# magicat777/Audio-Analyzer-OMEGA

Hardware: AMD Instinct MI355X
Metric: audio frames/sec (multi-res FFT + LUFS + TruePeak) at 1/2/4/8 MI355X (higher is better)
Workload: dtype f32; 1 GPU; cfg2: 256 stereo frames x 16384 samples per GPU; MRFFT 16k/8k/4k/1k + combine(512) + K-weighted LUFS + 4x true peak + meter aggregates; channel_frames_per_gpu=512, frame_samples=16384, target_bins=512, parallelism=frames sharded over 1 GPU(s)

## Files before the change

audio-analyzer-omega_amd/csrc/capi_batch.cpp:

```cpp

#include "batch_plan.hpp"
#include "host.hpp"

namespace {

constexpr int kChunkFrames = kMeterChunk;

int get_kw_tab(omega_ctx* c, int M, int L, BiquadTab** out) {
  const auto key = std::make_pair(M, L);
  auto it = c->kw_tabs.find(key);
  if (it != c->kw_tabs.end()) {
    *out = it->second;
    return 0;
  }
  const double fs = c->cfg.sample_rate;
  std::vector<BiquadTab> t = {make_biquad_tab(butter2(38.0, fs, true), L),
                              make_biquad_tab(butter2(1500.0, fs, true), L)};
  BiquadTab* d = nullptr;
  int r = upload(c, &d, t);
  if (r) return r;
  c->kw_tabs[key] = d;
  *out = d;
  return 0;
}
int get_kw_tab(omega_ctx* c, int M, BiquadTab** out) { return get_kw_tab(c, M, kw_chunk(M), out); }

hipError_t tp_launch(int W, const SpectralParams& sp, hipStream_t s) {
  if (W == 16384 || W == 8192) return launch_truepeak_rf(W, sp, s);
  return launch_truepeak(W, sp, s);
}

SpectralParams spectral_params(omega_ctx* c) {
  SpectralParams p{};
  p.tp_phases = 0xE;
  p.C = c->cfg.n_channels;
  p.n_res = c->cfg.n_res;
  p.rf_sizes = c->rf_sizes;
  for (int r = 0; r < p.n_res; ++r) {
    ResParam& q = p.res[r];
    q.n = c->cfg.res[r].fft_size;
    q.offset = c->cfg.frame_size - q.n;
    q.win = c->d_win[r];
    q.wgt = c->d_wgt[r];
    q.ent_begin = c->ent_begin[r];
    q.ent_end = c->ent_end[r];
    q.cw = (float)c->cfg.res[r].weight;
    q.low_band = c->ent_jmax[r] < 256;
    q.pair_lo = c->pair_lo[r];
    q.pair_hi = c->pair_hi[r];
  }
  p.ent = c->d_ent;
  p.T = c->cfg.target_bins;
  p.rot = c->d_rot;
  for (int l = 0; l < kMaxLog2; ++l) p.tw[l] = c->d_tw[l];
  return p;
}

bool aligned8(const void* p) { return ((uintptr_t)p & 7) == 0; }

std::vector<MeterPrepParams> meter_chunks(omega_ctx* c, const float* lufs, const float* tp, int64_t n_frames,
                                          double* out) {
  const int C = c->cfg.n_channels;
  std::vector<MeterPrepParams> v;
  for (int64_t f0 = 0; f0 < n_frames; f0 += kChunkFrames) {
    const int64_t nf = std::min<int64_t>(kChunkFrames, n_frames - f0);
    const int a = c->cur, b = c->cur ^ 1;
    MeterPrepParams p{};
    p.lufs = lufs + f0 * C;
    p.tp = tp + f0 * C;
    p.n_frames = nf;
    p.C = C;
    p.hist_l_in = c->d_hist_l[a];
    p.hist_t_in = c->d_hist_t[a];
    p.n_l_in = c->d_nl[a];
    p.n_t_in = c->d_nt[a];
    p.skeys_in = c->d_skeys[a];
    p.n_s_in = c->d_ns[a];
    p.t0_in = c->d_t0[a];
    p.hist_l_out = c->d_hist_l[b];
    p.hist_t_out = c->d_hist_t[b];
    p.n_l_out = c->d_nl[b];
    p.n_t_out = c->d_nt[b];
    p.skeys_out = c->d_skeys[b];
    p.n_s_out = c->d_ns[b];
    p.t0_out = c->d_t0[b];
    p.HL = c->HL;
    p.HT = c->HT;
    p.mom_len = c->cfg.momentary_len;
    p.short_len = c->cfg.short_len;
    p.int_len = c->cfg.integrated_len;
    p.peak_len = c->cfg.peak_len;
    p.poll_limit = c->poll_limit;
    p.err_word = c->d_err;
    p.gate = (float)c->cfg.gate_lufs;
    p.core = c->d_core[a];
    p.ext = c->d_ext[a];
    p.n_core = c->d_ncore[a];
    p.n_ext = c->d_next[a];
    p.gcount = c->d_gcount[a];
    p.gsum = c->d_gsum[a];
// ... 836 lines not shown
```

audio-analyzer-omega_amd/csrc/host.hpp:

```cpp
#pragma once

#include <hip/hip_runtime.h>

#include <algorithm>
#include <cmath>
#include <complex>
#include <cstdarg>
#include <cstdio>
#include <cstdlib>
#include <cstring>
#include <exception>
#include <map>
#include <new>
#include <string>
#include <vector>

#include "../../include/omega.h"
#include "design.hpp"
#include "params.hpp"

namespace omega {
hipError_t launch_mrfft(const SpectralParams& p, hipStream_t s);
hipError_t launch_mrfft_independent(const SpectralParams& p, hipStream_t s);
hipError_t launch_truepeak(int W, const SpectralParams& p, hipStream_t s);
// ... 188 lines not shown
  bool use_graph = false;
  int layout = 3;
  unsigned* d_kw_done = nullptr;
  unsigned kw_issued = 0;
  unsigned q_issued = 0;
  unsigned tp_issued = 0;
  unsigned prep_issued = 0;
  unsigned seg_issued = 0;
  unsigned lt_issued = 0;
  unsigned* tp_count_to = nullptr;
  bool side_meters = false;
  unsigned seg_par[2] = {0, 0};
  bool pipe = false;
  bool pend = false;
  MeterPrepParams pend_mq{};
  int pend_nq = 0, pend_par = 0;
  int stage_par = 0;
  unsigned* d_tail = nullptr;
  unsigned tail_issued = 0;
  unsigned long long* d_mirror = nullptr;
  unsigned mirror_gen = 0;
  int tail_ok = 0;
  hipStream_t bs[2] = {nullptr, nullptr};
  hipEvent_t ev_in = nullptr, ev_done[2] = {nullptr, nullptr};
  unsigned bs_idx = 0;
  int last_bs = 0;
  bool unjoined = false;
  bool bs_shared = false;
  std::vector<std::pair<const char*, size_t>> prev_span;
  unsigned* h_err = nullptr;
  unsigned* d_err = nullptr;
  int poll_limit = 1 << 22;
  float* d_lufs_scr = nullptr;
  int64_t lufs_scr_cap = 0;
  bool res_independent = false;
  hipEvent_t ev_kw = nullptr;
  struct GraphEntry {
    std::vector<uint64_t> key;
    hipGraph_t graph;
    hipGraphExec_t exec;
  };
  std::vector<GraphEntry> graphs;
  char err[512] = {};
  float2* d_tw[kMaxLog2] = {};

  float2* d_rot = nullptr;
  float* d_win[kMaxRes] = {};
  float* d_wgt[kMaxRes] = {};
  CombEnt* d_ent = nullptr;
  int ent_begin[kMaxRes] = {}, ent_end[kMaxRes] = {};
  int pair_lo[kMaxRes] = {}, pair_hi[kMaxRes] = {};
  int ent_jmax[kMaxRes] = {};
  std::map<std::pair<int, int>, BiquadTab*> kw_tabs;
  int rf_sizes = 1 << 14;
  std::map<std::pair<int, int>, float*> windows;
  std::map<int, float2*> rots;
  std::map<std::pair<int, int>, float4*> wgens;
  int* d_own_off = nullptr;
  int* d_own_rj = nullptr;
  float* d_own_frac = nullptr;
  std::map<int, std::pair<double*, std::pair<int, int>>> chroma_mats;
  double chroma_df = 0.0;
  struct ChromaTab {
    int n_bins = 0, lo = 0, hi = 0;
    double df = 0.0;
    float4* w4 = nullptr;
    float* w1 = nullptr;
    unsigned short* perm = nullptr;
    int* goff = nullptr;
    float* rec = nullptr;
  } ctab;
  int n_cu = 0;
  DrumState drum;
  PostState post;
  VuState vu;
  TransientState tr;
  PitchState pitch;
  HarmonicState harm;
  GenreState genre;
  HipHopState hiphop;
  PhaseState phase;
  RoomState room;
  VoiceState voice;
  TdetectState tdetect;
  BassZoomState basszoom;
  W64Stage* w64[4] = {};
  struct AnyPlan {
    std::vector<int> radix;
    float2* tw = nullptr;
    double2* tw64 = nullptr;
    float2* rot = nullptr;
  };
  std::map<int, AnyPlan> any_plans;
  float2* d_any = nullptr;
  int64_t any_cap = 0;
  double* d_w64 = nullptr;
  int64_t w64_cap = 0;
  float* d_hist_l[2] = {};
  float* d_hist_t[2] = {};
  int* d_nl[2] = {};
  int* d_nt[2] = {};
  int cur = 0;
  unsigned long long* d_skeys[2] = {};
  int* d_ns[2] = {};
  uint32_t* d_t0[2] = {};
  float* d_core[2] = {nullptr, nullptr};
  MeterExt* d_ext[2] = {nullptr, nullptr};
// ... 275 lines not shown
```

audio-analyzer-omega_amd/csrc/params.hpp:

```cpp
#pragma once
#include <hip/hip_runtime.h>
#include <stdint.h>

namespace omega {

constexpr int kMaxRes = 4;
constexpr int kMaxLog2 = 15;

__device__ __forceinline__ float tp_db(float peak) {
  return peak < 1e-10f ? -100.0f : (float)(20.0 * log10((double)peak));
}

struct alignas(16) CombEnt {
  int tm, j;
  float c0, c1;
};

struct ResParam {
  int n;
  int offset;
  const float* win;
  const float* wgt;
  float* mag_out;
  int ent_begin, ent_end;
  float cw;
  int low_band;
  int pair_lo, pair_hi;
};

struct SpectralParams {
  const float* x;
  int64_t frame_stride, chan_stride;
  int C;
  int64_t n_cf;
  int n_res;
  ResParam res[kMaxRes];
  const CombEnt* ent;
  int T;
  float* comb_out;
  float* tp_out;
  const float2* rot;
  int tp_phases;
  const float2* tw[kMaxLog2];
  int rf_sizes;
  unsigned* tp_done;
  float* tp_copy;
};

struct BiquadTab {
  float b0, a1, a2, B0, B1;
  float zi0, zi1;
  float h0[64], h1[64];
  float pw[64][4];
  float g0[64], g1[64];
};

constexpr int kPwl = 96;
constexpr int kw_threads(int M) { return M / 32 < 64 ? 64 : (M / 32 > 512 ? 512 : M / 32); }
constexpr int kw_chunk(int M) { return M / kw_threads(M); }

struct KWeightParams {
  const float* x;
  int64_t frame_stride, chan_stride;
  int C;
  int64_t n_cf;
  const BiquadTab* hp;
  const BiquadTab* shelf;
  float* lufs_out;
  float* weighted_out;
// ... 537 lines not shown
```

audio-analyzer-omega_amd/csrc/regfft.hpp:

```cpp
#pragma once
#include "fft.hpp"

namespace omega {

__device__ constexpr float kCos128[16] = {
    1.000000000e+00f, 9.987954562e-01f, 9.951847267e-01f, 9.891765100e-01f, 9.807852804e-01f,
    9.700312532e-01f, 9.569403357e-01f, 9.415440652e-01f, 9.238795325e-01f, 9.039892931e-01f,
    8.819212643e-01f, 8.577286100e-01f, 8.314696123e-01f, 8.032075315e-01f, 7.730104534e-01f,
    7.409511254e-01f};
__device__ constexpr float kSin128[16] = {
    0.000000000e+00f, 4.906767433e-02f, 9.801714033e-02f, 1.467304745e-01f, 1.950903220e-01f,
    2.429801799e-01f, 2.902846773e-01f, 3.368898534e-01f, 3.826834324e-01f, 4.275550934e-01f,
    4.713967368e-01f, 5.141027442e-01f, 5.555702330e-01f, 5.956993045e-01f, 6.343932842e-01f,
    6.715589548e-01f};

__device__ __forceinline__ void wave_lds_sync() {
  asm volatile("s_waitcnt lgkmcnt(0)" ::: "memory");
  __builtin_amdgcn_wave_barrier();
}

__device__ __forceinline__ float lane_xor1(float v) {
  return __int_as_float(__builtin_amdgcn_mov_dpp(__float_as_int(v), 0xB1, 0xF, 0xF, true));
}

// ... 123 lines not shown
    }
  }
  static __device__ __forceinline__ void twiddle_t2(float2 (&v)[16], const float2* t2u) {
    static_for<1, 16>([&](auto k2) { v[k2] = cmul(v[k2], t2u[(k2 - 1) * L]); });
  }

  template <bool SYNC = false, bool LT2 = false>
  static __device__ __forceinline__ void run(float2 (&v)[16], float2* buf, int t, float2 w1, float2 w2,
                                             const float2* t2 = nullptr) {
    run2<SYNC, LT2>(v, buf, t, t, w1, w2, t2);
  }
  template <bool SYNC = false, bool LT2 = false>
  static __device__ __forceinline__ void run2(float2 (&v)[16], float2* buf, int t1, int t, float2 w1, float2 w2,
                                              const float2* t2 = nullptr) {
    dft16(v);
    twiddle(v, w1);
    if constexpr (SYNC) __syncthreads();
    {
      float2* b = buf + t1;
      static_for<0, 16>([&](auto k1) { b[P1 * k1] = v[k1]; });
    }
    __syncthreads();
    {
      const int u = t % L, k1 = t / L;
      const float2* b = buf + P1 * k1 + u;
      static_for<0, 16>([&](auto r) { v[r] = b[L * r]; });
      dft16(v);
      if constexpr (LT2)
        twiddle_t2(v, t2 + u);
      else
        twiddle(v, w2);
      float2* bw = buf + P2R * k1 + u;
      static_for<0, 16>([&](auto k2) { bw[P2C * k2] = v[k2]; });
    }
    wave_lds_sync();
    if constexpr (L == 16) {
      const int k2 = t & 15, k1 = t >> 4;
      const float2* b = buf + P2R * k1 + P2C * k2;
      static_for<0, 16>([&](auto r) { v[r] = b[r]; });
      dft16(v);
    } else {
      const int q = t & 1, k2 = (t >> 1) & 15, k1 = t >> 5;
      const float2* b = buf + P2R * k1 + P2C * k2 + q;
      static_for<0, 16>([&](auto r) { v[r] = b[2 * r]; });
      dft16(v);
      static_for<0, 16>([&](auto m) {
        const float2 tw = twc<m + 16, 32>(v[m]);
        v[m] = make_float2(q ? tw.x : v[m].x, q ? tw.y : v[m].y);
      });
      lane_pair_fmac(v, q ? 1.f : -1.f);
    }
  }

  template <bool SYNC = false, bool LT2 = false>
  static __device__ __forceinline__ void run_low(float2 (&v)[16], float2* buf, int t, float2 w1, float2 w2,
                                                 const float2* t2 = nullptr) {
    static_assert(L == 32, "the two-band pass 3 is the K = 8192 plan");
    dft16(v);
    twiddle(v, w1);
    if constexpr (SYNC) __syncthreads();
    {
      float2* b = buf + t;
      static_for<0, 16>([&](auto k1) { b[P1 * k1] = v[k1]; });
    }
    __syncthreads();
    {
      const int u = t % L, k1 = t / L;
      const float2* b = buf + P1 * k1 + u;
      static_for<0, 16>([&](auto r) { v[r] = b[L * r]; });
      dft16(v);
      if constexpr (LT2)
        twiddle_t2(v, t2 + u);
      else
        twiddle(v, w2);
      float2* bw = buf + P2R * k1 + u;
      static_for<0, 16>([&](auto k2) { bw[P2C * k2] = v[k2]; });
    }
    wave_lds_sync();
    const int q = t & 1, k2 = (t >> 1) & 15, k1 = t >> 5;
    {
      const float2* b = buf + P2R * k1 + P2C * k2 + q;
      static_for<0, 16>([&](auto r) { v[r] = b[2 * r]; });
    }
    float2 f0 = v[0], f15 = v[0];
    static_for<1, 16>([&](auto r) {
      f0 = cadd(f0, v[r]);
      f15 = cadd(f15, twc<15 * r, 16>(v[r]));
    });
    const float2 g = twc<15, 32>(f15);
    const float2 send = q ? f0 : f15;
    const float2 recv = make_float2(lane_xor1(send.x), lane_xor1(send.y));
    const float2 out = q ? csub(recv, g) : cadd(f0, recv);
    __syncthreads();
    buf[s3o(t) + (q ? o3o(15) : 0)] = out;
    __syncthreads();
  }

  template <bool LT2 = false>
  static __device__ __forceinline__ void run_half(float2 (&v)[16], float* bf, int t, float2 w1, float2 w2,
                                                  const float2* t2 = nullptr) {
    static_assert(L == 16, "the half-buffer plan is K = 4096");
    dft16(v);
    twiddle(v, w1);
    const int u = t % L, k1 = t / L;
    {
      float* b = bf + t;
      static_for<0, 16>([&](auto j) { b[P1 * j] = v[j].x; });
    }
    __syncthreads();
    {
      const float* b = bf + P1 * k1 + u;
      static_for<0, 16>([&](auto r) { v[r].x = b[L * r]; });
    }
    __syncthreads();
    {
      float* b = bf + t;
      static_for<0, 16>([&](auto j) { b[P1 * j] = v[j].y; });
    }
    __syncthreads();
    {
      const float* b = bf + P1 * k1 + u;
      static_for<0, 16>([&](auto r) { v[r].y = b[L * r]; });
    }
    dft16(v);
    if constexpr (LT2)
      twiddle_t2(v, t2 + u);
    else
      twiddle(v, w2);
    {
      float* bw = bf + P2R * k1 + u;
      static_for<0, 16>([&](auto j) { bw[P2C * j] = v[j].x; });
    }
    wave_lds_sync();
    const int k2 = t & 15, k1b = t >> 4;
    const float* br = bf + P2R * k1b + P2C * k2;
    static_for<0, 16>([&](auto r) { v[r].x = br[r]; });
    {
      float* bw = bf + P2R * k1 + u;
      static_for<0, 16>([&](auto j) { bw[P2C * j] = v[j].y; });
    }
    wave_lds_sync();
    static_for<0, 16>([&](auto r) { v[r].y = br[r]; });
    dft16(v);
  }
  template <bool IM>
  static __device__ __forceinline__ void store_spectrum_half(const float2 (&v)[16], float* bf, int t) {
    float* b = bf + s3o(t);
    static_for<0, 16>([&](auto m) { b[o3o(m)] = IM ? v[m].y : v[m].x; });
// ... 10 lines not shown
```

audio-analyzer-omega_amd/csrc/rfkern.hip:

```cpp
#include <cstdlib>

#include "stamps.hpp"

namespace omega {
OMEGA_STAMPS_DECL
OMEGA_WGTRACE_DECL
OMEGA_MARKS_DECL
}

#include "kw.hpp"
#include "meter_query.hpp"
#include "regfft.hpp"
#include "spectral.hpp"

namespace omega {

template <int K>
constexpr size_t t2_offset() { return (RegFFT<K>::kSlots + 8) * sizeof(float2) + 64; }
template <int K>
constexpr size_t lds_bytes() { return t2_offset<K>() + RegFFT<K>::kT2 * sizeof(float2); }
template <int K>
__device__ __forceinline__ float2* t2_table(char* smem) { return reinterpret_cast<float2*>(smem + t2_offset<K>()); }

template <int NTH>
// ... 81 lines not shown
      const float2 a = bo[FFT::o3(r)];
      float2 b = bm[FFT::o3(15 - r)];
      if constexpr (K == 8192 && r == 8) {
        if (t == 0) b = a;
      }
      float2 xk, xkk;
      untangle(a, b, twc<r, 32>(wm), xk, xkk);
      if constexpr (r == 0) {
        if (t == 0) {
          xn = a.x - a.y;
          xk = make_float2(a.x + a.y, 0.f);
        }
      }
      v[r] = xk;
    });
  }
  float2 y[16];
  static_for<0, 16>([&](auto r) { y[r] = v[r]; });
  const float2 hz = make_float2(wm.y, wm.x);
  float fmx = 0.f;
  const int lane = tid & 63;
  const int mir_addr = 4 * ((t == 0 || t == NTH / 2) ? lane : lane ^ 63);
  OMEGA_STAMP(4);
#pragma unroll 1
  for (int P = 1; P <= 3; ++P) {
    int tl = t, tidl = tid;
    float2 w1l = w1, w2l = w2, rhol = rho, hzl = hz;
    asm volatile("" : "+v"(tl), "+v"(tidl), "+v"(w1l.x), "+v"(w1l.y), "+v"(w2l.x), "+v"(w2l.y));
    asm volatile("" : "+v"(rhol.x), "+v"(rhol.y), "+v"(hzl.x), "+v"(hzl.y));
    static_for<0, 16>([&](auto r) {
      const float2 rk = cmul(rhol, make_float2(kCos128[r], kSin128[r]));
      y[r] = cmul(y[r], rk);
    });
    if (!((p.tp_phases >> P) & 1)) continue;
    OMEGA_STAMP(1 + 4 * P);
    const float cp = P == 1 ? 7.071067812e-01f : (P == 2 ? 0.f : -7.071067812e-01f);
    OMEGA_STAMP(2 + 4 * P);
    static_for<0, 16>([&](auto r) {
      const float2 m = y[15 - r];
      float2 yp = make_float2(__int_as_float(__builtin_amdgcn_ds_bpermute(mir_addr, __float_as_int(m.x))),
                              -__int_as_float(__builtin_amdgcn_ds_bpermute(mir_addr, __float_as_int(m.y))));
      if constexpr (r == 0) {
        if (tl == 0) yp = make_float2(xn * cp, 0.f);
      } else {
        if (tl == 0) yp = cconj(y[16 - r]);
      }
      const float2 g = twc<-r, 32>(hzl);
      const float2 S = cadd(y[r], yp), D = csub(y[r], yp);
      v[r] = make_float2(fmaf(g.x, D.x, fmaf(-g.y, D.y, S.x)), fmaf(-g.x, D.y, fmaf(-g.y, D.x, -S.y)));
    });
    OMEGA_STAMP(3 + 4 * P);
    FFT::template run2<true, true>(v, buf, tl, tidl, w1l, w2l, t2);
    max3_abs16(fmx, v);
#if defined(OMEGA_EXP_STALL)
    asm volatile("s_sleep %0" ::"i"(OMEGA_EXP_STALL));
#endif
#if defined(OMEGA_EXP_VALU)
    {
      float d0 = fmx, d1 = mx, d2 = fmx + 1.f, d3 = mx + 1.f;
      asm volatile(".rept %4\n v_fma_f32 %0, %0, %5, %6\n v_fma_f32 %1, %1, %5, %6\n"
                   " v_fma_f32 %2, %2, %5, %6\n v_fma_f32 %3, %3, %5, %6\n .endr"
                   : "+v"(d0), "+v"(d1), "+v"(d2), "+v"(d3)
                   : "i"(OMEGA_EXP_VALU), "v"(0.5f), "v"(0.25f));
    }
#endif
    OMEGA_STAMP(4 + 4 * P);
  }
  const float peak = block_max<NTH>(fmaxf(mx, fmx * (0.5f / K)), red, tid);
  if (tid == 0) {
    const float db = tp_db(peak);
    if (p.tp_done) {
      __hip_atomic_store(reinterpret_cast<unsigned*>(p.tp_out + cf), __float_as_uint(db), __ATOMIC_RELAXED,
                         __HIP_MEMORY_SCOPE_AGENT);
      asm volatile("s_waitcnt vmcnt(0)" ::: "memory");
      __hip_atomic_fetch_add(p.tp_done, 1u, __ATOMIC_RELAXED, __HIP_MEMORY_SCOPE_AGENT);
    } else {
      p.tp_out[cf] = db;
    }
    if (p.tp_copy) p.tp_copy[cf] = db;
  }
}

template <int K>
__global__ __launch_bounds__(K / 16, 4) void truepeak_rf_kernel(SpectralParams p) {
  extern __shared__ __attribute__((aligned(16))) char smem[];
  OMEGA_WG_BEGIN();
  truepeak_rf_body<K>(p, blockIdx.x, threadIdx.x, smem);
  OMEGA_WG_END(1);
}

template <int K>
__device__ __forceinline__ void mrfft_rf_body(const SpectralParams& p, int r, int64_t cf, int t, char* smem) {
  using FFT = RegFFT<K>;
  constexpr int NTH = FFT::NTH, M = 2 * K;
  float2* buf = reinterpret_cast<float2*>(smem);
  const int64_t f = cf / p.C, c = cf % p.C;
  const ResParam& rp = p.res[r];
  const float2* x2 = reinterpret_cast<const float2*>(p.x + f * p.frame_stride + c * p.chan_stride + rp.offset);
  const float2* __restrict__ twK = p.tw[ilog2(K)];
  const float2* __restrict__ twM = p.tw[ilog2(M)];
  float2 v[16];
  const float2 w1 = twK[t], w2b = twK[16 * (t % FFT::L)];
  const float2 wm = twM[t];
  float2* t2 = t2_table<K>(smem);
  FFT::fill_t2(t2, twK, t);
  asm volatile("" ::: "memory");
  const float2* w2 = reinterpret_cast<const float2*>(rp.win);
  static_for<0, 16>([&](auto q) {
    const float2 a = x2[t + NTH * q], w = w2[t + NTH * q];
    v[q] = make_float2(a.x * w.x, a.y * w.y);
  });
  const int e0 = rp.ent_begin + t;
  CombEnt ent{};
  if (p.comb_out && e0 < rp.ent_end) ent = p.ent[e0];
  bool low = false;
  if constexpr (K == 8192) low = !rp.mag_out && rp.low_band;
  if (low) {
    if constexpr (K == 8192) FFT::template run_low<false, true>(v, buf, t, w1, w2b, t2);
  } else {
    FFT::template run<false, true>(v, buf, t, w1, w2b, t2);
    __syncthreads();
    FFT::store_spectrum(v, buf, t);
    __syncthreads();
  }
  if (!rp.mag_out) {
    if (!p.comb_out) return;
    auto mag_at = [&](int j) -> float {
      const float2 a = buf[FFT::a3(j == K ? 0 : j)];
      if (j == 0) return fabsf(a.x + a.y);
      if (j == K) return fabsf(a.x - a.y);
      if (j == K / 2) return cabs(a);
      const float2 b = buf[FFT::a3(K - j)];
      float2 xk, xkk;
      untangle(a, b, twM[j], xk, xkk);
      return cabs(xk);
    };
    float* o = p.comb_out + cf * p.T;
    auto apply = [&](const CombEnt& en) {
      const int tt = en.tm & 0xFFFFFF, op = en.tm >> 24;
      if (op == 2) {
        o[tt] = 0.f;
        return;
      }
      const float val = fmaf(en.c1, mag_at(en.j + 1), en.c0 * mag_at(en.j));
      if (op == 0)
        o[tt] = val;
      else
        o[tt] += val;
    };
    if (e0 < rp.ent_end) apply(ent);
    for (int e = e0 + NTH; e < rp.ent_end; e += NTH) apply(p.ent[e]);
    return;
  }
  float mg[16];
  float mnyq = 0.f;
  {
    const float2* bo = buf + FFT::s3(t);
    const float2* bm = buf + FFT::s3m(t);
    static_for<0, 16>([&](auto q) {
      const float2 a = bo[FFT::o3(q)];
      float2 b = bm[FFT::o3(15 - q)];
      if constexpr (K == 8192 && q == 8) {
        if (t == 0) b = a;
      }
      float2 xk, xkk;
      untangle(a, b, twc<q, 32>(wm), xk, xkk);
      mg[q] = cabs(xk);
      if constexpr (q == 0) {
        if (t == 0) {
          mg[0] = fabsf(a.x + a.y);
          mnyq = fabsf(a.x - a.y);
        }
      }
    });
  }
  if (rp.mag_out) {
    float* o = rp.mag_out + cf * (K + 1);
    const float* __restrict__ wgt = rp.wgt;
    static_for<0, 16>([&](auto q) { o[t + NTH * q] = mg[q] * wgt[t + NTH * q]; });
    if (t == 0) o[K] = mnyq * wgt[K];
  }
  if (!p.comb_out) return;
  float* mag = reinterpret_cast<float*>(smem);
  __syncthreads();
  static_for<0, 16>([&](auto q) { mag[t + NTH * q] = mg[q]; });
  if (t == 0) mag[K] = mnyq;
  __syncthreads();
  float* o = p.comb_out + cf * p.T;
  auto apply = [&](const CombEnt& en) {
    const int tt = en.tm & 0xFFFFFF, op = en.tm >> 24;
    const float val = fmaf(en.c1, mag[en.j + 1], en.c0 * mag[en.j]);
    if (op == 0)
      o[tt] = val;
    else if (op == 1)
      o[tt] += val;
    else
      o[tt] = 0.f;
  };
  if (e0 < rp.ent_end) apply(ent);
  for (int e = e0 + NTH; e < rp.ent_end; e += NTH) apply(p.ent[e]);
}

template <int K>
__global__ __launch_bounds__(K / 16, 4) void mrfft_rf_kernel(SpectralParams p, int r) {
  extern __shared__ __attribute__((aligned(16))) char smem[];
  OMEGA_WG_BEGIN();
  mrfft_rf_body<K>(p, r, blockIdx.x, threadIdx.x, smem);
  OMEGA_WG_END(2);
}

OMEGA_STAMPS_GETTER(omega_debug_rf_stamps)
OMEGA_WGTRACE_GETTER(omega_debug_wgtrace)
OMEGA_MARKS_GETTER(omega_debug_marks_batch)

hipError_t launch_mrfft_rf(int n, const SpectralParams& p, int r, hipStream_t s) {
  const dim3 grid((unsigned)p.n_cf);
  if (n == 16384) {
    hipLaunchKernelGGL(mrfft_rf_kernel<8192>, grid, dim3(512), lds_bytes<8192>(), s, p, r);
  } else if (n == 8192) {
    hipLaunchKernelGGL(mrfft_rf_kernel<4096>, grid, dim3(256), lds_bytes<4096>(), s, p, r);
  } else {
    return hipErrorInvalidValue;
  }
  return hipGetLastError();
}

constexpr int kSpecRfThreads = 256;
#ifndef OMEGA_SPEC_WGS
#define OMEGA_SPEC_WGS 5
#endif
constexpr int kSpecRfWgs = OMEGA_SPEC_WGS;
constexpr int kSpecRfPeakWords = 12;
template <int K>
struct SpecRfLds {
  static constexpr size_t kT2Off = RegFFT<K>::kSlots * sizeof(float);
  static constexpr size_t kXform = kT2Off + RegFFT<K>::kT2 * sizeof(float2);
  static constexpr size_t kPartOff = ((K + 1) * sizeof(float) + 15) / 16 * 16;
  static constexpr size_t kClsOff = kPartOff + 240 * 5 * sizeof(float);
  static constexpr size_t kRedOff = kClsOff + 12 * 5 * sizeof(double);
  static constexpr size_t kFlagOff = (kRedOff + (RegFFT<K>::NTH / 64) * sizeof(float) + 15) / 16 * 16;
  static constexpr int kFlagWords = 2 * 64 * kSpecRfPeakWords / 4;
  static constexpr size_t kPost = kFlagOff + kFlagWords * sizeof(unsigned);
  static constexpr size_t kBytes = kXform > kPost ? kXform : kPost;
  static_assert((kBytes + 1279) / 1280 * 1280 * kSpecRfWgs <= 160 * 1024, "LDS of kSpecRfWgs workgroups per CU");
};


template <int K>
__device__ __forceinline__ void spectra_rf_body(const SpectraParams& p) {
  using FFT = RegFFT<K>;
  constexpr int NTH = FFT::NTH;
  static_assert(NTH == kSpecRfThreads, "one 256-thread workgroup per frame");
  extern __shared__ __attribute__((aligned(16))) char smem[];
  using Lds = SpecRfLds<K>;
  float* bf = reinterpret_cast<float*>(smem);
  float* magc = reinterpret_cast<float*>(smem);
  constexpr int kFlagWords = Lds::kFlagWords;
  float* part = reinterpret_cast<float*>(smem + Lds::kPartOff);
  double(*cls)[5] = reinterpret_cast<double(*)[5]>(smem + Lds::kClsOff);
  float* redf = reinterpret_cast<float*>(smem + Lds::kRedOff);
// ... 245 lines not shown
    const double chm = cls[cm][0] + cls[cm][1] + cls[cm][2] + cls[cm][3] + cls[cm][4];
    const double chp = cls[cp][0] + cls[cp][1] + cls[cp][2] + cls[cp][3] + cls[cp][4];
    const double sm = 0.25 * chm + 0.5 * ch + 0.25 * chp;
    double tot = t < 12 ? sm : 0.0;
    tot += __shfl_xor(tot, 8, 64);
    tot += __shfl_xor(tot, 4, 64);
    tot += __shfl_xor(tot, 2, 64);
    tot += __shfl_xor(tot, 1, 64);
    if (t < 12) p.chroma_out[fr * 12 + c] = tot > 0 ? sm / tot : sm;
  }
  OMEGA_STAMP(11);
  OMEGA_STAMP_RT(31);
}

template <int K>
__global__ __launch_bounds__(kSpecRfThreads, kSpecRfWgs) void spectra_rf_kernel(SpectraParams p) {
  OMEGA_WG_BEGIN();
  spectra_rf_body<K>(p);
  OMEGA_WG_END(20);
}

hipError_t launch_spectra_rf(int m, const SpectraParams& p, hipStream_t s) {
  if (m != 8192 || (p.chroma_out && p.c_hi > 2 * 64 * kSpecRfPeakWords)) return hipErrorInvalidValue;
  hipLaunchKernelGGL(spectra_rf_kernel<4096>, dim3((unsigned)p.n), dim3(kSpecRfThreads), SpecRfLds<4096>::kBytes,
                     s, p);
  return hipGetLastError();
}

hipError_t launch_truepeak_rf(int W, const SpectralParams& p, hipStream_t s, int extra_lds) {
  const dim3 grid((unsigned)p.n_cf);
  if (W == 16384) {
    hipLaunchKernelGGL(truepeak_rf_kernel<8192>, grid, dim3(512), lds_bytes<8192>() + extra_lds, s, p);
  } else if (W == 8192) {
    hipLaunchKernelGGL(truepeak_rf_kernel<4096>, grid, dim3(256), lds_bytes<4096>(), s, p);
  } else {
    return hipErrorInvalidValue;
  }
  return hipGetLastError();
}

constexpr int kBatchThreads = 512;

template <int K>
__device__ __forceinline__ void batch_multi(const SpectralParams& p, int r, int64_t wg, int tid, float2* smem) {
  constexpr int G = threads_for<K>();
  constexpr int FPW = kBatchThreads / G;
  static_assert(FPW * K * sizeof(float2) <= lds_bytes<8192>(), "LDS of one batch workgroup");
  const int grp = tid / G;
  const int64_t cf = wg * FPW + grp;
  const bool valid = cf < p.n_cf;
  mrfft_frame<K, G>(p, r, valid ? cf : p.n_cf - 1, valid, tid % G, smem + grp * K);
}

__device__ __forceinline__ void batch_kw_role(const KWeightParams& kp, int64_t cf, int tid, char* smem) {
  constexpr int kP = 2 * kPwl * 16;
  auto* pwl = reinterpret_cast<float4(*)[kPwl]>(smem);
  float* fbuf = reinterpret_cast<float*>(smem + kP);
  float* sh = reinterpret_cast<float*>(smem + kP + 65536);
  float* edge = sh + 36;
  double* red = reinterpret_cast<double*>(smem + kP + 65536 + 224);
  static_assert(kP + 65536 + 224 + 64 <= lds_bytes<8192>(), "K-weighting role LDS");
  kweight_body<16384, kBatchThreads, true, true>(kp, cf, tid, pwl, fbuf, sh, edge, red);
  kw_count_in(kp, tid);
}

__device__ __forceinline__ void batch_meter_role(const MeterPrepParams& mp, int q, int nq, int tid) {
  const int64_t n_out = mp.n_frames * mp.C, step = (int64_t)nq * (kBatchThreads / 64);
  const int64_t o0 = (int64_t)q * (kBatchThreads / 64) + (tid >> 6);
  const int lane = tid & 63;
  OMEGA_MARK(q, 0);
  if (tid == 0) poll_count(mp.start_ctr, mp.start_target, mp.poll_limit, mp.err_word + 1);
  __syncthreads();
  OMEGA_MARK(q, 1);
  for (int64_t o = o0; o < n_out; o += step) meter_query_wave(mp, o / mp.C, (int)(o % mp.C), lane, true, false);
  const float th0 = o0 < n_out ? tp_hist_part(mp, o0 / mp.C, (int)(o0 % mp.C), lane) : -INFINITY;
  OMEGA_MARK(q, 2);
  if (tid == 0) poll_count(mp.join_ctr, mp.join_target, mp.poll_limit, mp.err_word + 1);
  __syncthreads();
  OMEGA_MARK(q, 3);
  const int64_t n_roll = (int64_t)mp.C * mp.HT, roll_step = (int64_t)nq * kBatchThreads;
  int64_t e = (int64_t)q * kBatchThreads + tid;
  float rv = 0.f;
  const int64_t rdst = e < n_roll ? tp_roll_load(mp, e, rv) : -1;
  for (int64_t o = o0; o < n_out; o += step) {
    const int64_t f = o / mp.C;
    const int c = (int)(o % mp.C);
    tp_finish(mp, f, c, lane, o == o0 ? th0 : tp_hist_part(mp, f, c, lane));
  }
  if (rdst >= 0) mp.hist_t_out[rdst] = rv;
  for (e += roll_step; e < n_roll; e += roll_step) {
    const int64_t d = tp_roll_load(mp, e, rv);
    if (d >= 0) mp.hist_t_out[d] = rv;
  }
  if (mp.seg_ctr) {
    asm volatile("s_waitcnt vmcnt(0)" ::: "memory");
    __syncthreads();
    if (tid == 0) __hip_atomic_fetch_add(mp.seg_ctr, 1u, __ATOMIC_RELAXED, __HIP_MEMORY_SCOPE_AGENT);
  }
  OMEGA_MARK(q, 4);
}

__device__ __forceinline__ void batch_body(const SpectralParams& sp, const KWeightParams& kp, const BatchPlan& bp,
                                           const MeterPrepParams& mq, char* smem) {
  const int tid = threadIdx.x;
  const int b = blockIdx.x;
  OMEGA_WG_BEGIN();
  if (bp.tail_ctr && b == (int)gridDim.x - 1 && tid == 0)
    __hip_atomic_fetch_add(bp.tail_ctr, 1u, __ATOMIC_RELAXED, __HIP_MEMORY_SCOPE_SYSTEM);
  if (b >= bp.q_begin && b < bp.q_begin + bp.q_n) {
    batch_meter_role(mq, b - bp.q_begin, bp.q_n, tid);
    OMEGA_WG_END(4);
    return;
  }

  const int len0 = bp.seg_begin[1], len1 = bp.seg_begin[2] - bp.seg_begin[1];
  const int sg = (b >= bp.seg_start[0] && b < bp.seg_start[0] + len0) ? 0
                 : (b >= bp.seg_start[1] && b < bp.seg_start[1] + len1) ? 1 : -1;
  if (sg >= 0) {
    const int j = b - bp.seg_start[sg], nr = bp.n_roles[sg];
    int role;
    int64_t cf;
    if (nr == 2 && bp.pat == 1) {
      const int g = j >> 3, per = g & 7, rb = (0x5A >> per) & 1;
      role = bp.roles[sg][rb];
      const int idx = 4 * (g >> 3) + __popc((rb ? 0x5A : 0xA5) & ((1 << per) - 1));
      cf = (int64_t)idx * 8 + (j & 7);
    } else {
      role = bp.roles[sg][(j >> 3) % nr];
      cf = (int64_t)(j / (8 * nr)) * 8 + (j & 7);
    }
    if (cf >= sp.n_cf) return;
    if (role == 0) {
      batch_kw_role(kp, cf, tid, smem);
    } else if (role == 1) {
      truepeak_rf_body<8192>(sp, cf, tid, smem);
    } else {
      mrfft_rf_body<8192>(sp, bp.mr_res, cf, tid, smem);
    }
    OMEGA_WG_END(role);
    return;
  }
  const MultiPlan& mp = bp.multi;
  const int w = b - bp.multi_start -
                (b >= bp.q_begin + bp.q_n && bp.q_begin < bp.multi_start + bp.multi_n ? bp.q_n : 0);
  if (w < 0 || w >= bp.multi_n) return;
  int s = 0;
  while (s + 1 < mp.n_seg && w >= mp.wg_begin[s + 1]) ++s;
  const int r = mp.res[s];
  const int64_t wg = w - mp.wg_begin[s];
  float2* buf = reinterpret_cast<float2*>(smem);
  switch (sp.res[r].n) {
    case 512: batch_multi<256>(sp, r, wg, tid, buf); break;
    case 1024: batch_multi<512>(sp, r, wg, tid, buf); break;
    case 2048: batch_multi<1024>(sp, r, wg, tid, buf); break;
    case 4096: batch_multi<2048>(sp, r, wg, tid, buf); break;
    case 8192: batch_multi<4096>(sp, r, wg, tid, buf); break;
    default: break;
  }
  OMEGA_WG_END(3 + sp.res[r].n);
}

__global__ __launch_bounds__(kBatchThreads, 4) void batch_kernel(SpectralParams sp, KWeightParams kp, BatchPlan bp,
                                                                 MeterPrepParams mq) {
  extern __shared__ __attribute__((aligned(16))) char smem[];
  batch_body(sp, kp, bp, mq, smem);
}

hipError_t launch_batch(const SpectralParams& sp, const KWeightParams& kp, const BatchPlan& bp, const MeterPrepParams& mq,
                        int grid, hipStream_t s) {
  hipLaunchKernelGGL(batch_kernel, dim3((unsigned)grid), dim3(kBatchThreads), lds_bytes<8192>(), s, sp, kp, bp, mq);
  return hipGetLastError();
}

}
```

audio-analyzer-omega_amd/csrc/spectral.hip:

```cpp
#include "stamps.hpp"

namespace omega {
OMEGA_STAMPS_DECL
}

#include "spectral.hpp"

namespace omega {

template <int K, int NTH = threads_for<K>()>
__global__ __launch_bounds__(NTH, 2 * NTH / 256) void mrfft_kernel(SpectralParams p, int r) {
  extern __shared__ __attribute__((aligned(16))) char smem[];
  mrfft_frame<K, NTH>(p, r, blockIdx.x, true, threadIdx.x, reinterpret_cast<float2*>(smem));
}

constexpr int kMultiThreads = 256;

template <int K>
__device__ __forceinline__ void mrfft_multi_seg(const SpectralParams& p, int r, int64_t wg, float2* smem) {
  constexpr int G = threads_for<K>();
  constexpr int FPW = kMultiThreads / G;
  const int grp = threadIdx.x / G;
  const int64_t cf = wg * FPW + grp;
  const bool valid = cf < p.n_cf;
  mrfft_frame<K, G>(p, r, valid ? cf : p.n_cf - 1, valid, threadIdx.x % G, smem + grp * K);
}

__global__ __launch_bounds__(kMultiThreads) void mrfft_multi_kernel(SpectralParams p, MultiPlan mp) {
  extern __shared__ __attribute__((aligned(16))) char smem[];
  float2* buf = reinterpret_cast<float2*>(smem);
  int s = 0;
  while (s + 1 < mp.n_seg && (int)blockIdx.x >= mp.wg_begin[s + 1]) ++s;
  const int r = mp.res[s];
  const int64_t wg = (int64_t)blockIdx.x - mp.wg_begin[s];
  switch (p.res[r].n) {
    case 512: mrfft_multi_seg<256>(p, r, wg, buf); break;
    case 1024: mrfft_multi_seg<512>(p, r, wg, buf); break;
    case 2048: mrfft_multi_seg<1024>(p, r, wg, buf); break;
    case 4096: mrfft_multi_seg<2048>(p, r, wg, buf); break;
    case 8192: mrfft_multi_seg<4096>(p, r, wg, buf); break;
    default: break;
  }
}

template <int K, int NTH = tp_threads<K>()>
__global__ __launch_bounds__(NTH, (NTH / 256 > 2 ? NTH / 256 : 2)) void truepeak_kernel(SpectralParams p) {
  extern __shared__ __attribute__((aligned(16))) char smem[];
  float2* bufA = reinterpret_cast<float2*>(smem);
  truepeak_body<K, NTH>(p, blockIdx.x, threadIdx.x, bufA, bufA + K, reinterpret_cast<float*>(smem + 2 * K * sizeof(float2)));
}

template <int K, int NTH = threads_for<K>()>
__global__ __launch_bounds__(NTH, 2 * NTH / 256) void rfft_kernel(RfftParams p) {
  using FFT = BlockFFT<K, NTH>;
  extern __shared__ __attribute__((aligned(16))) char smem[];
  float2* buf = reinterpret_cast<float2*>(smem);
  const int tid = threadIdx.x;
  const int64_t i = blockIdx.x;
  const float2* x2 = reinterpret_cast<const float2*>(p.x + i * (2 * K));
  const float2* w2 = reinterpret_cast<const float2*>(p.win);
  FFT::run_from(buf, FFT::load_tw(p.tw[ilog2(K)], tid), tid, [&](int n) {
    const float2 a = x2[n], w = w2[n];
    return make_float2(a.x * w.x, a.y * w.y);
  });
  const float2* __restrict__ twN = p.tw[ilog2(2 * K)];
  float2* cp = p.cplx ? reinterpret_cast<float2*>(p.cplx) + i * (K + 1) : nullptr;
  float* mp = p.mag ? p.mag + i * (K + 1) : nullptr;
  for (int k = tid; k < K / 2; k += NTH) {
    float2 xk, xkk;
    if (k == 0) {
      const float2 z = buf[FFT::out(0)];
      xk = make_float2(z.x + z.y, 0.f);
      xkk = make_float2(z.x - z.y, 0.f);
      const float2 xm = cconj(buf[FFT::out(K / 2)]);
      if (cp) cp[K / 2] = xm;
      if (mp) mp[K / 2] = cabs(xm);
    } else {
      untangle(buf[FFT::out(k)], buf[FFT::out(K - k)], twN[k], xk, xkk);
    }
    if (cp) {
      cp[k] = xk;
      cp[K - k] = xkk;
    }
    if (mp) {
      mp[k] = cabs(xk);
      mp[K - k] = cabs(xkk);
    }
  }
}

__global__ __launch_bounds__(256) void combine_kernel(CombineParams p) {
  const int64_t cf = blockIdx.y;
  for (int t = blockIdx.x * 256 + threadIdx.x; t < p.T; t += gridDim.x * 256) {
// ... 68 lines not shown
  }

hipError_t launch_mrfft_rf(int n, const SpectralParams& p, int r, hipStream_t s);

hipError_t launch_mrfft_range(const SpectralParams& p, int r0, int r1, hipStream_t s) {
  const dim3 grid((unsigned)p.n_cf);
  for (int r = r0; r < r1 && r < p.n_res; ++r) {
    if (!p.comb_out && !p.res[r].mag_out) continue;
    if (p.res[r].n < 512) {
      hipLaunchKernelGGL(mrfft_small_kernel, grid, dim3(kSmallThreads), 0, s, p, r);
      const hipError_t e = hipGetLastError();
      if (e != hipSuccess) return e;
      continue;
    }
    if ((p.rf_sizes >> ilog2(p.res[r].n)) & 1) {
      const hipError_t e = launch_mrfft_rf(p.res[r].n, p, r, s);
      if (e != hipSuccess) return e;
      continue;
    }
#define OMEGA_RES(K) \
  hipLaunchKernelGGL(mrfft_kernel<K>, grid, dim3(threads_for<K>()), K * sizeof(float2), s, p, r)
    OMEGA_SWITCH_K(p.res[r].n, OMEGA_RES)
#undef OMEGA_RES
    const hipError_t e = hipGetLastError();
    if (e != hipSuccess) return e;
  }
  return hipSuccess;
}

OMEGA_STAMPS_GETTER(omega_debug_spectral_stamps)

hipError_t launch_truepeak(int W, const SpectralParams& p, hipStream_t s) {
  const dim3 grid((unsigned)p.n_cf);
  if (p.tp_out) {
#define OMEGA_TP(K) \
  (void)hipFuncSetAttribute(reinterpret_cast<const void*>(&truepeak_kernel<K>), \
                            hipFuncAttributeMaxDynamicSharedMemorySize, 2 * K * sizeof(float2) + 16 * sizeof(float)); \
  hipLaunchKernelGGL(truepeak_kernel<K>, grid, dim3(tp_threads<K>()), 2 * K * sizeof(float2) + 16 * sizeof(float), \
                     s, p)
    OMEGA_SWITCH_K(W, OMEGA_TP)
#undef OMEGA_TP
  }
  return hipGetLastError();
}

hipError_t launch_mrfft(const SpectralParams& p, hipStream_t s) { return launch_mrfft_range(p, 0, p.n_res, s); }

hipError_t launch_mrfft_independent(const SpectralParams& p, hipStream_t s) {
  MultiPlan mp{};
  int nwg = 0;
  for (int r = 0; r < p.n_res; ++r) {
    if (!p.comb_out && !p.res[r].mag_out) continue;
    const int n = p.res[r].n;
    if (n > 8192 || n < 512 || ((p.rf_sizes >> ilog2(n)) & 1)) {
      const hipError_t e = launch_mrfft_range(p, r, r + 1, s);
      if (e != hipSuccess) return e;
      continue;
    }
    const int K = n / 2;
    const int G = K / 16 < 64 ? 64 : K / 16;
    const int fpw = kMultiThreads / G;
    mp.res[mp.n_seg] = r;
    mp.wg_begin[mp.n_seg] = nwg;
    ++mp.n_seg;
    nwg += (int)((p.n_cf + fpw - 1) / fpw);
  }
  if (mp.n_seg == 0) return hipSuccess;
  hipLaunchKernelGGL(mrfft_multi_kernel, dim3((unsigned)nwg), dim3(kMultiThreads), 4096 * sizeof(float2), s, p, mp);
  return hipGetLastError();
}

hipError_t launch_spectral(int W, const SpectralParams& p, hipStream_t s) {
  const hipError_t e = launch_mrfft(p, s);
  return e != hipSuccess ? e : launch_truepeak(W, p, s);
}

hipError_t launch_combine(const CombineParams& p, hipStream_t s) {
  hipLaunchKernelGGL(combine_kernel, dim3((unsigned)((p.T + 255) / 256), (unsigned)p.n_cf), dim3(256), 0, s, p);
  return hipGetLastError();
}

hipError_t launch_rfft(int m, const RfftParams& p, hipStream_t s) {
  const dim3 grid((unsigned)p.n);
#define OMEGA_RF(K) hipLaunchKernelGGL(rfft_kernel<K>, grid, dim3(threads_for<K>()), K * sizeof(float2), s, p)
  OMEGA_SWITCH_K(m, OMEGA_RF)
#undef OMEGA_RF
  return hipGetLastError();
}

}
```

Before: 8.658 million channel-frames/s.

## Route 8k-point resolution through register FFT with low-band pass and two frames per workgroup

Moves the 8192-sample resolution off the generic shared-memory multi-frame FFT onto the register-based RegFFT<4096> path. It generalises the low-band last pass to the L==16 plan, which computes only the bins the combine needs, and packs two frames per batch workgroup with separate twiddle tables. It also removes leftover stall and VALU experiment hooks. The aim is fewer LDS round trips and less work for the low-band-only case, at the cost of a new code path, extra LDS per workgroup and possible occupancy changes.

```diff
diff --git a/audio-analyzer-omega_amd/csrc/capi_batch.cpp b/audio-analyzer-omega_amd/csrc/capi_batch.cpp
--- a/audio-analyzer-omega_amd/csrc/capi_batch.cpp
+++ b/audio-analyzer-omega_amd/csrc/capi_batch.cpp
@@ -45,7 +45,7 @@
     q.ent_begin = c->ent_begin[r];
     q.ent_end = c->ent_end[r];
     q.cw = (float)c->cfg.res[r].weight;
-    q.low_band = c->ent_jmax[r] < 256;
+    q.low_band = c->ent_jmax[r] < kLowBandBins;
     q.pair_lo = c->pair_lo[r];
     q.pair_hi = c->pair_hi[r];
   }
diff --git a/audio-analyzer-omega_amd/csrc/host.hpp b/audio-analyzer-omega_amd/csrc/host.hpp
--- a/audio-analyzer-omega_amd/csrc/host.hpp
+++ b/audio-analyzer-omega_amd/csrc/host.hpp
@@ -264,7 +264,7 @@
   int pair_lo[kMaxRes] = {}, pair_hi[kMaxRes] = {};
   int ent_jmax[kMaxRes] = {};
   std::map<std::pair<int, int>, BiquadTab*> kw_tabs;
-  int rf_sizes = 1 << 14;
+  int rf_sizes = (1 << 14) | (1 << 13);
   std::map<std::pair<int, int>, float*> windows;
   std::map<int, float2*> rots;
   std::map<std::pair<int, int>, float4*> wgens;
diff --git a/audio-analyzer-omega_amd/csrc/params.hpp b/audio-analyzer-omega_amd/csrc/params.hpp
--- a/audio-analyzer-omega_amd/csrc/params.hpp
+++ b/audio-analyzer-omega_amd/csrc/params.hpp
@@ -15,6 +15,8 @@
   int tm, j;
   float c0, c1;
 };
+
+constexpr int kLowBandBins = 256;
 
 struct ResParam {
   int n;
diff --git a/audio-analyzer-omega_amd/csrc/regfft.hpp b/audio-analyzer-omega_amd/csrc/regfft.hpp
--- a/audio-analyzer-omega_amd/csrc/regfft.hpp
+++ b/audio-analyzer-omega_amd/csrc/regfft.hpp
@@ -199,10 +199,11 @@
     }
   }
 
+  static constexpr int kLowBand = 256;
+
   template <bool SYNC = false, bool LT2 = false>
   static __device__ __forceinline__ void run_low(float2 (&v)[16], float2* buf, int t, float2 w1, float2 w2,
                                                  const float2* t2 = nullptr) {
-    static_assert(L == 32, "the two-band pass 3 is the K = 8192 plan");
     dft16(v);
     twiddle(v, w1);
     if constexpr (SYNC) __syncthreads();
@@ -224,23 +225,48 @@
       static_for<0, 16>([&](auto k2) { bw[P2C * k2] = v[k2]; });
     }
     wave_lds_sync();
-    const int q = t & 1, k2 = (t >> 1) & 15, k1 = t >> 5;
-    {
-      const float2* b = buf + P2R * k1 + P2C * k2 + q;
-      static_for<0, 16>([&](auto r) { v[r] = b[2 * r]; });
-    }
-    float2 f0 = v[0], f15 = v[0];
-    static_for<1, 16>([&](auto r) {
-      f0 = cadd(f0, v[r]);
-      f15 = cadd(f15, twc<15 * r, 16>(v[r]));
-    });
-    const float2 g = twc<15, 32>(f15);
-    const float2 send = q ? f0 : f15;
-    const float2 recv = make_float2(lane_xor1(send.x), lane_xor1(send.y));
-    const float2 out = q ? csub(recv, g) : cadd(f0, recv);
-    __syncthreads();
-    buf[s3o(t) + (q ? o3o(15) : 0)] = out;
-    __syncthreads();
+    if constexpr (L == 16) {
+      {
+        const int k2 = t & 15, k1 = t >> 4;
+        const float2* b = buf + P2R * k1 + P2C * k2;
+        static_for<0, 16>([&](auto r) { v[r] = b[r]; });
+      }
+      float2 lo[16], hi[16];
+      static_for<0, 16>([&](auto r) {
+        lo[r] = v[r];
+        hi[r] = twc<15 * r, 16>(v[r]);
+      });
+      static_for<0, 4>([&](auto s) {
+        constexpr int h = 8 >> s;
+        static_for<0, h>([&](auto i) {
+          lo[i] = cadd(lo[i], lo[i + h]);
+          hi[i] = cadd(hi[i], hi[i + h]);
+        });
+      });
+      __syncthreads();
+      float2* o = buf + s3o(t);
+      o[0] = lo[0];
+      o[o3o(15)] = hi[0];
+      __syncthreads();
+    } else {
+      const int q = t & 1, k2 = (t >> 1) & 15, k1 = t >> 5;
+      {
+        const float2* b = buf + P2R * k1 + P2C * k2 + q;
+        static_for<0, 16>([&](auto r) { v[r] = b[2 * r]; });
+      }
+      float2 f0 = v[0], f15 = v[0];
+      static_for<1, 16>([&](auto r) {
+        f0 = cadd(f0, v[r]);
+        f15 = cadd(f15, twc<15 * r, 16>(v[r]));
+      });
+      const float2 g = twc<15, 32>(f15);
+      const float2 send = q ? f0 : f15;
+      const float2 recv = make_float2(lane_xor1(send.x), lane_xor1(send.y));
+      const float2 out = q ? csub(recv, g) : cadd(f0, recv);
+      __syncthreads();
+      buf[s3o(t) + (q ? o3o(15) : 0)] = out;
+      __syncthreads();
+    }
   }
 
   template <bool LT2 = false>
diff --git a/audio-analyzer-omega_amd/csrc/rfkern.hip b/audio-analyzer-omega_amd/csrc/rfkern.hip
--- a/audio-analyzer-omega_amd/csrc/rfkern.hip
+++ b/audio-analyzer-omega_amd/csrc/rfkern.hip
@@ -157,18 +157,6 @@
     OMEGA_STAMP(3 + 4 * P);
     FFT::template run2<true, true>(v, buf, tl, tidl, w1l, w2l, t2);
     max3_abs16(fmx, v);
-#if defined(OMEGA_EXP_STALL)
-    asm volatile("s_sleep %0" ::"i"(OMEGA_EXP_STALL));
-#endif
-#if defined(OMEGA_EXP_VALU)
-    {
-      float d0 = fmx, d1 = mx, d2 = fmx + 1.f, d3 = mx + 1.f;
-      asm volatile(".rept %4\n v_fma_f32 %0, %0, %5, %6\n v_fma_f32 %1, %1, %5, %6\n"
-                   " v_fma_f32 %2, %2, %5, %6\n v_fma_f32 %3, %3, %5, %6\n .endr"
-                   : "+v"(d0), "+v"(d1), "+v"(d2), "+v"(d3)
-                   : "i"(OMEGA_EXP_VALU), "v"(0.5f), "v"(0.25f));
-    }
-#endif
     OMEGA_STAMP(4 + 4 * P);
   }
   const float peak = block_max<NTH>(fmaxf(mx, fmx * (0.5f / K)), red, tid);
@@ -195,7 +183,8 @@
 }
 
 template <int K>
-__device__ __forceinline__ void mrfft_rf_body(const SpectralParams& p, int r, int64_t cf, int t, char* smem) {
+__device__ __forceinline__ void mrfft_rf_body(const SpectralParams& p, int r, int64_t cf, int t, char* smem, float2* t2,
+                                              bool valid = true) {
   using FFT = RegFFT<K>;
   constexpr int NTH = FFT::NTH, M = 2 * K;
   float2* buf = reinterpret_cast<float2*>(smem);
@@ -207,7 +196,6 @@
   float2 v[16];
   const float2 w1 = twK[t], w2b = twK[16 * (t % FFT::L)];
   const float2 wm = twM[t];
-  float2* t2 = t2_table<K>(smem);
   FFT::fill_t2(t2, twK, t);
   asm volatile("" ::: "memory");
   const float2* w2 = reinterpret_cast<const float2*>(rp.win);
@@ -218,10 +206,10 @@
   const int e0 = rp.ent_begin + t;
   CombEnt ent{};
   if (p.comb_out && e0 < rp.ent_end) ent = p.ent[e0];
-  bool low = false;
-  if constexpr (K == 8192) low = !rp.mag_out && rp.low_band;
+  static_assert(FFT::kLowBand == kLowBandBins, "ResParam::low_band is stated for RegFFT::run_low's bands");
+  const bool low = !rp.mag_out && rp.low_band;
   if (low) {
-    if constexpr (K == 8192) FFT::template run_low<false, true>(v, buf, t, w1, w2b, t2);
+    FFT::template run_low<false, true>(v, buf, t, w1, w2b, t2);
   } else {
     FFT::template run<false, true>(v, buf, t, w1, w2b, t2);
     __syncthreads();
@@ -229,7 +217,7 @@
     __syncthreads();
   }
   if (!rp.mag_out) {
-    if (!p.comb_out) return;
+    if (!p.comb_out || !valid) return;
     auto mag_at = [&](int j) -> float {
       const float2 a = buf[FFT::a3(j == K ? 0 : j)];
       if (j == 0) return fabsf(a.x + a.y);
@@ -279,7 +267,7 @@
       }
     });
   }
-  if (rp.mag_out) {
+  if (rp.mag_out && valid) {
     float* o = rp.mag_out + cf * (K + 1);
     const float* __restrict__ wgt = rp.wgt;
     static_for<0, 16>([&](auto q) { o[t + NTH * q] = mg[q] * wgt[t + NTH * q]; });
@@ -291,6 +279,7 @@
   static_for<0, 16>([&](auto q) { mag[t + NTH * q] = mg[q]; });
   if (t == 0) mag[K] = mnyq;
   __syncthreads();
+  if (!valid) return;
   float* o = p.comb_out + cf * p.T;
   auto apply = [&](const CombEnt& en) {
     const int tt = en.tm & 0xFFFFFF, op = en.tm >> 24;
@@ -310,7 +299,7 @@
 __global__ __launch_bounds__(K / 16, 4) void mrfft_rf_kernel(SpectralParams p, int r) {
   extern __shared__ __attribute__((aligned(16))) char smem[];
   OMEGA_WG_BEGIN();
-  mrfft_rf_body<K>(p, r, blockIdx.x, threadIdx.x, smem);
+  mrfft_rf_body<K>(p, r, blockIdx.x, threadIdx.x, smem, t2_table<K>(smem));
   OMEGA_WG_END(2);
 }
 
@@ -662,6 +651,19 @@
   mrfft_frame<K, G>(p, r, valid ? cf : p.n_cf - 1, valid, tid % G, smem + grp * K);
 }
 
+__device__ __forceinline__ void batch_res8k(const SpectralParams& p, int r, int64_t wg, int tid, char* smem) {
+  using FFT = RegFFT<4096>;
+  constexpr int G = FFT::NTH;
+  static_assert(kBatchThreads == 2 * G, "two 256-thread halves");
+  constexpr size_t kBuf = (FFT::kSlots + 8) * sizeof(float2), kTab = FFT::kT2 * sizeof(float2);
+  static_assert(2 * (kBuf + kTab) <= lds_bytes<8192>(), "LDS of one batch workgroup");
+  const int grp = tid / G;
+  const int64_t cf = wg * 2 + grp;
+  const bool valid = cf < p.n_cf;
+  mrfft_rf_body<4096>(p, r, valid ? cf : p.n_cf - 1, tid % G, smem + grp * kBuf,
+                      reinterpret_cast<float2*>(smem + 2 * kBuf + grp * kTab), valid);
+}
+
 __device__ __forceinline__ void batch_kw_role(const KWeightParams& kp, int64_t cf, int tid, char* smem) {
   constexpr int kP = 2 * kPwl * 16;
   auto* pwl = reinterpret_cast<float4(*)[kPwl]>(smem);
@@ -745,7 +747,7 @@
     } else if (role == 1) {
       truepeak_rf_body<8192>(sp, cf, tid, smem);
     } else {
-      mrfft_rf_body<8192>(sp, bp.mr_res, cf, tid, smem);
+      mrfft_rf_body<8192>(sp, bp.mr_res, cf, tid, smem, t2_table<8192>(smem));
     }
     OMEGA_WG_END(role);
     return;
@@ -764,7 +766,7 @@
     case 1024: batch_multi<512>(sp, r, wg, tid, buf); break;
     case 2048: batch_multi<1024>(sp, r, wg, tid, buf); break;
     case 4096: batch_multi<2048>(sp, r, wg, tid, buf); break;
-    case 8192: batch_multi<4096>(sp, r, wg, tid, buf); break;
+    case 8192: batch_res8k(sp, r, wg, tid, smem); break;
     default: break;
   }
   OMEGA_WG_END(3 + sp.res[r].n);
diff --git a/audio-analyzer-omega_amd/csrc/spectral.hip b/audio-analyzer-omega_amd/csrc/spectral.hip
--- a/audio-analyzer-omega_amd/csrc/spectral.hip
+++ b/audio-analyzer-omega_amd/csrc/spectral.hip
@@ -38,7 +38,6 @@
     case 1024: mrfft_multi_seg<512>(p, r, wg, buf); break;
     case 2048: mrfft_multi_seg<1024>(p, r, wg, buf); break;
     case 4096: mrfft_multi_seg<2048>(p, r, wg, buf); break;
-    case 8192: mrfft_multi_seg<4096>(p, r, wg, buf); break;
     default: break;
   }
 }
@@ -213,7 +212,7 @@
   for (int r = 0; r < p.n_res; ++r) {
     if (!p.comb_out && !p.res[r].mag_out) continue;
     const int n = p.res[r].n;
-    if (n > 8192 || n < 512 || ((p.rf_sizes >> ilog2(n)) & 1)) {
+    if (n > 4096 || n < 512 || ((p.rf_sizes >> ilog2(n)) & 1)) {
       const hipError_t e = launch_mrfft_range(p, r, r + 1, s);
       if (e != hipSuccess) return e;
       continue;
```

Result: no change. 8.673 million channel-frames/s (median of 4 runs) (+0.2%).
